# gmongaras/Stable-Diffusion-3-From-Scratch

Measured on AMD Instinct MI355X. Metric: train images/sec MMDiT-B 256^2 bf16, higher is better.
Workload: dtype bf16

## Files before the change

### stable-diffusion-3-from-scratch_amd/csrc/rowops.hip

```cpp
#include "common.h"
#include <float.h>

namespace {

constexpr float LN_EPS = 1e-5f;
constexpr float RMS_EPS = FLT_EPSILON;

__device__ __forceinline__ float bf16_round(float x) { return __builtin_bit_cast(float, pack_bf2(x, 0.f) << 16); }

template <int NITX, typename TO, typename TA, bool RES, bool MX = false>
__device__ __forceinline__ void ln_mod_fwd_body(int block, const float* __restrict__ x, const float* __restrict__ scale, const float* __restrict__ shift,
                                                int64_t ld_mod, int rows, int d, int rpb, TO* __restrict__ out,
                                                float* __restrict__ mean_o, float* __restrict__ rstd_o,
                                                const TA* __restrict__ acc, const float* __restrict__ gate, int64_t ld_gate, float* __restrict__ xo,
                                                unsigned char* __restrict__ mx_scales) {
  constexpr int NIT = NITX < 0 ? -NITX : NITX;
  constexpr bool EXACT = NITX < 0;
  const int lane = threadIdx.x & 63, row = block * 4 + (threadIdx.x >> 6);
  if (row >= rows) return;
  const int nch = d >> 2;
  const int b = row / rpb;
  const float* xr = x + (int64_t)row * d;
  float v[NIT][4];
  float s = 0.f;
// ... 194 lines not shown
    flush(dh, dshift + (int64_t)b * ld_dmod);
    if constexpr (GATED) {
      flush(sg, dgate + (int64_t)b * ld_dgate);
      if (dbias) flush(sb, dbias + (int64_t)b * ld_dbias);
    }
  }
}

struct LnBwdProb {
  const void* dout; const float* x; const float* mean; const float* rstd; const float* scale; int64_t ld_mod; const float* dres; int rpb, nchunk;
  float* dx; float* dscale; float* dshift; int64_t ld_dmod;
  const void* acc; const float* gate; int64_t ld_gate; void* dacc; float* dgate; int64_t ld_dgate; float* dbias; int64_t ld_dbias;
};
template <int NIT, typename TG, typename TA, bool GATED>
__global__ __launch_bounds__(256) void ln_mod_bwd_kernel(LnBwdProb p0, LnBwdProb p1, int nblk0, int d, int rch) {
  const bool first = (int)blockIdx.x < nblk0;
  const LnBwdProb& p = first ? p0 : p1;
  ln_mod_bwd_body<NIT, TG, TA, GATED>(first ? (int)blockIdx.x : (int)blockIdx.x - nblk0, (const TG*)p.dout, p.x, p.mean, p.rstd, p.scale, p.ld_mod, p.dres, d, p.rpb, p.nchunk,
                                      p.dx, p.dscale, p.dshift, p.ld_dmod, (const TA*)p.acc, p.gate, p.ld_gate, (TA*)p.dacc, p.dgate, p.ld_dgate, p.dbias, p.ld_dbias, rch);
}

template <int NITX, typename TI, typename TO>
__global__ __launch_bounds__(256) void text_rms_fwd_kernel(const TI* __restrict__ x, const float* __restrict__ w, const float* __restrict__ sp,
                                                           int rows, int cnt, int tokens, int off, int d, TO* __restrict__ out) {
  constexpr int NIT = NITX < 0 ? -NITX : NITX;
  constexpr bool EXACT = NITX < 0;
  const int lane = threadIdx.x & 63, m = blockIdx.x * 4 + (threadIdx.x >> 6);
  if (m >= rows) return;
  const int nch = d >> 2;
  const TI* xr = x + ((int64_t)(m / cnt) * tokens + off + m % cnt) * d;
  float v[NIT][4];
  float q = 0.f;
#pragma unroll
  for (int it = 0; it < NIT; it++) {
    int ch = lane + 64 * it;
    if (EXACT || ch < nch) { ld4(xr + ch * 4, v[it]); q += v[it][0] * v[it][0] + v[it][1] * v[it][1] + v[it][2] * v[it][2] + v[it][3] * v[it][3]; }
  }
  const float rinv = rsqrtf(wave_sum(q) / d + RMS_EPS);
  const float s = sp[0];
  TO* orow = out + (int64_t)m * d;
#pragma unroll
  for (int it = 0; it < NIT; it++) {
    int ch = lane + 64 * it;
    if (EXACT || ch < nch) {
      float wv[4], o[4];
      ld4(w + ch * 4, wv);
#pragma unroll
      for (int e = 0; e < 4; e++) o[e] = s * (v[it][e] * rinv * wv[e]);
      st4(orow + ch * 4, o);
    }
  }
}

#ifndef TRB_ROWS
#define TRB_ROWS 64
#endif
struct TextRmsBwdHalf { const void* dout; const float* w; const float* sp; int rows, cnt, off; float* dw; float* dsp; };
template <int NITX, typename TI, typename TG>
__global__ __launch_bounds__(512) void text_rms_bwd_kernel(TextRmsBwdHalf h0, TextRmsBwdHalf h1, const TI* __restrict__ x, int tokens, int d) {
  constexpr int NIT = NITX < 0 ? -NITX : NITX;
  constexpr bool EXACT = NITX < 0;
  const TextRmsBwdHalf& hp = blockIdx.y == 0 ? h0 : h1;
  const TG* __restrict__ dout = (const TG*)hp.dout;
  const float* __restrict__ w = hp.w;
  const float* __restrict__ sp = hp.sp;
  const int rows = hp.rows, cnt = hp.cnt, off = hp.off;
  float* __restrict__ dw = hp.dw;
  float* __restrict__ dsp = hp.dsp;
  __shared__ float red[NIT * 256];
  for (int c = threadIdx.x; c < NIT * 256; c += 512) red[c] = 0.f;
  __syncthreads();
  const int lane = threadIdx.x & 63, wave = threadIdx.x >> 6;
  const int nch = d >> 2;
  const float s = sp[0];
  float accw[NIT][4], wv[NIT][4];
  float accs = 0.f;
#pragma unroll
  for (int it = 0; it < NIT; it++) {
    int ch = lane + 64 * it;
    if (EXACT || ch < nch) ld4(w + ch * 4, wv[it]); else { wv[it][0] = wv[it][1] = wv[it][2] = wv[it][3] = 0.f; }
#pragma unroll
    for (int e = 0; e < 4; e++) accw[it][e] = 0.f;
  }
  for (int m = blockIdx.x * TRB_ROWS + wave; m < min(rows, (int)(blockIdx.x + 1) * TRB_ROWS); m += 8) {
    const TI* xr = x + ((int64_t)(m / cnt) * tokens + off + m % cnt) * d;
    float v[NIT][4];
    float q = 0.f;
#pragma unroll
    for (int it = 0; it < NIT; it++) {
      int ch = lane + 64 * it;
      if (EXACT || ch < nch) { ld4(xr + ch * 4, v[it]); q += v[it][0] * v[it][0] + v[it][1] * v[it][1] + v[it][2] * v[it][2] + v[it][3] * v[it][3]; }
    }
    const float rinv = rsqrtf(wave_sum(q) / d + RMS_EPS);
#pragma unroll
    for (int it = 0; it < NIT; it++) {
      int ch = lane + 64 * it;
      if (EXACT || ch < nch) {
        float dy[4];
        ld4(dout + (int64_t)m * d + ch * 4, dy);
#pragma unroll
        for (int e = 0; e < 4; e++) { float xn = v[it][e] * rinv; accw[it][e] += dy[e] * s * xn; accs += dy[e] * xn * wv[it][e]; }
      }
    }
  }
#pragma unroll
  for (int it = 0; it < NIT; it++) {
    const int ch = lane + 64 * it;
    if (EXACT || ch < nch) {
#pragma unroll
      for (int e = 0; e < 4; e++) atomicAdd(&red[ch * 4 + e], accw[it][e]);
    }
  }
  __syncthreads();
#ifndef TRB_NO_GLOBAL
  for (int c = threadIdx.x; c < d; c += 512) atomicAdd(dw + c, red[c]);
#else
  if (red[threadIdx.x] == 123.456f) dw[0] = 1.f;
#endif
  accs = wave_sum(accs);
#ifndef TRB_NO_DSP
  if (lane == 0) atomicAdd(dsp, accs);
#else
  if (accs == 123.456f) dsp[0] = 1.f;
#endif
}

__device__ __forceinline__ float group8_sum(float v) {
  v += __shfl_xor(v, 1, 64); v += __shfl_xor(v, 2, 64); v += __shfl_xor(v, 4, 64);
  return v;
}

template <typename TI>
__device__ __forceinline__ void qk_norm_rope_fwd_body(int bid, int rstride, const TI* __restrict__ qkv, const float* __restrict__ wq, const float* __restrict__ wk,
                                                      const float* __restrict__ rcos, const float* __restrict__ rsin,
                                                      int rows, int tokens, int heads, int s_total, int tok0,
                                                      bf16_t* __restrict__ Q, bf16_t* __restrict__ K, bf16_t* __restrict__ V) {
  const int hc = threadIdx.x % (8 * heads), part = threadIdx.x / (8 * heads), head = hc >> 3, chunk = hc & 7;
  bf16_t* obase = part == 0 ? Q : part == 1 ? K : V;
  float w[8];
#pragma unroll
  for (int e = 0; e < 8; e++) w[e] = 0.f;
  if (part < 2) ld8((part == 0 ? wq : wk) + chunk * 8, w);
  const bool same_token = rcos && rstride % tokens == 0;
  float cs[2][8], sn[2][8];
  if (same_token && part < 2) {
    const int n = bid % tokens;
    ld8(rcos + (int64_t)n * 64 + chunk * 8, cs[0]);
    ld8(rsin + (int64_t)n * 64 + chunk * 8, sn[0]);
#pragma unroll
    for (int e = 0; e < 8; e++) { cs[1][e] = cs[0][e]; sn[1][e] = sn[0][e]; }
  }
  for (int row0 = bid; row0 < rows; row0 += 2 * rstride) {
    float x[2][8];
#pragma unroll
    for (int k = 0; k < 2; k++) {
      const int row = min(row0 + k * rstride, rows - 1);
      ld8(qkv + (((int64_t)row * 3 + part) * heads + head) * 64 + chunk * 8, x[k]);
    }
    if (part < 2 && rcos && !same_token) {
#pragma unroll
      for (int k = 0; k < 2; k++) {
        const int n = min(row0 + k * rstride, rows - 1) % tokens;
        ld8(rcos + (int64_t)n * 64 + chunk * 8, cs[k]);
        ld8(rsin + (int64_t)n * 64 + chunk * 8, sn[k]);
      }
    }
#pragma unroll
    for (int k = 0; k < 2; k++) {
      const int row = row0 + k * rstride;
      if (row >= rows) break;
      const int n = row % tokens, b = row / tokens;
      if (part < 2) {
        float ss = 0.f;
#pragma unroll
        for (int e = 0; e < 8; e++) ss += x[k][e] * x[k][e];
        const float rinv = rsqrtf(group8_sum(ss) * (1.f / 64.f) + RMS_EPS);
#pragma unroll
// ... 216 lines not shown
        ld8_nt(qkv + ((((int64_t)pr * 2 + k) * 3 + part) * heads + head) * 64 + chunk * 8, x[k]);
        if (rcos) {
          ld8(rcos + (int64_t)(2 * j + k) * 64 + chunk * 8, cs[k]);
          ld8(rsin + (int64_t)(2 * j + k) * 64 + chunk * 8, sn[k]);
        }
      }
#pragma unroll
      for (int k = 0; k < 2; k++) {
        float ss = 0.f;
#pragma unroll
        for (int e = 0; e < 8; e++) ss += x[k][e] * x[k][e];
        const float rinv = rsqrtf(group8_sum(ss) * (1.f / 64.f) + RMS_EPS);
        if (rcos) {
#pragma unroll
          for (int p = 0; p < 4; p++) {
            float da = dz[k][2 * p], db = dz[k][2 * p + 1];
            dz[k][2 * p] = da * cs[k][2 * p] + db * sn[k][2 * p + 1];
            dz[k][2 * p + 1] = db * cs[k][2 * p + 1] - da * sn[k][2 * p];
          }
        }
        float dot = 0.f;
#pragma unroll
        for (int e = 0; e < 8; e++) {
          float xh = x[k][e] * rinv;
          aw[e] += dz[k][e] * xh;
          dz[k][e] *= w[e];
          dot += dz[k][e] * xh;
          x[k][e] = xh;
        }
        dot = group8_sum(dot) * (1.f / 64.f);
#pragma unroll
        for (int e = 0; e < 8; e++) dz[k][e] = rinv * (dz[k][e] - x[k][e] * dot);
      }
    }
#pragma unroll
    for (int k = 0; k < 2; k++) st8(dqkv + ((((int64_t)pr * 2 + k) * 3 + part) * heads + head) * 64 + chunk * 8, dz[k]);
  }
  if (part < 2) {
#pragma unroll
    for (int e = 0; e < 8; e++) atomicAdd(&sdw[part][chunk * 8 + e], aw[e]);
  }
  __syncthreads();
  for (int i = threadIdx.x; i < 128; i += blockDim.x) atomicAdd((i < 64 ? dwq : dwk) + (i & 63), sdw[i >> 6][i & 63]);
}
template <typename TG, typename TI, typename TO>
__global__ __launch_bounds__(512) void qk_merge_bwd_kernel(QkProb p0, QkProb p1, int g0, int heads, int s_total) {
  const bool first = (int)blockIdx.x < g0;
  const QkProb& p = first ? p0 : p1;
  qk_merge_bwd_body<TG, TI, TO>(first ? (int)blockIdx.x : (int)blockIdx.x - g0, first ? g0 : (int)gridDim.x - g0, (const TG*)p.dQ, (const TG*)p.dK, (const TG*)p.dV,
                                (const TI*)p.qkv, p.wq, p.wk, p.rcos, p.rsin, p.rows >> 1, p.tokens, heads, s_total, p.tok0, (TO*)p.dqkv, p.dwq, p.dwk);
}

constexpr int CO_RCH = 64;

__device__ __forceinline__ float gelu_f(float x) { return 0.5f * x * (1.f + erff(x * 0.70710678118654752440f)); }
__device__ __forceinline__ float gelu_grad_f(float x) {
  return 0.5f * (1.f + erff(x * 0.70710678118654752440f)) + x * 0.39894228040143267794f * __expf(-0.5f * x * x);
}

template <typename T, bool GELU, bool MX = false>
__global__ __launch_bounds__(256) void mlp_act_fwd_kernel(const T* __restrict__ gu, T* __restrict__ h, int rows, int hidden, unsigned char* __restrict__ mx_scales = nullptr) {
  const int tx = threadIdx.x & 31, ty = threadIdx.x >> 5;
  const int c = blockIdx.x * 256 + tx * 8;
  if (c >= hidden) return;
  const int64_t ldi = GELU ? hidden : 2 * (int64_t)hidden;
  const int rend = min(rows, (int)(blockIdx.y + 1) * CO_RCH);
  for (int r0 = blockIdx.y * CO_RCH + ty; r0 < rend; r0 += 16) {
    float g[2][8], u[2][8];
#pragma unroll
    for (int k = 0; k < 2; k++) {
      const int r = r0 + 8 * k;
      if (r < rend) {
        ld8(gu + r * ldi + c, g[k]);
        if constexpr (!GELU) ld8(gu + r * ldi + hidden + c, u[k]);
      }
    }
#pragma unroll
    for (int k = 0; k < 2; k++) {
      const int r = r0 + 8 * k;
      if (r >= rend) break;
      float o[8];
#pragma unroll
      for (int e = 0; e < 8; e++) o[e] = GELU ? gelu_f(g[k][e]) : silu_f(g[k][e]) * u[k][e];
      if constexpr (MX) {
        float amax = 0.f;
#pragma unroll
        for (int e = 0; e < 8; e++) { o[e] = bf16_round(o[e]); amax = fmaxf(amax, fabsf(o[e])); }
        amax = fmaxf(amax, __shfl_xor(amax, 1, 64));
        amax = fmaxf(amax, __shfl_xor(amax, 2, 64));
        float inv;
        const int ex = mx_exponent(amax, inv);
        *(uint2*)((unsigned char*)h + (int64_t)r * hidden + c) = make_uint2(mx_pack4(o, inv), mx_pack4(o + 4, inv));
        if ((tx & 3) == 0) mx_scales[mx_scale_index(r, c >> 5, rows)] = (unsigned char)(ex + 127);
      } else {
        st8(h + (int64_t)r * hidden + c, o);
      }
    }
  }
}

__device__ __forceinline__ void colsum_flush(float (&acc)[8], float* sbuf , float* dst, int c, int ncols) {
  const int tx = threadIdx.x & 127, ty = threadIdx.x >> 7;
  if (ty == 1) {
#pragma unroll
    for (int e = 0; e < 8; e++) sbuf[tx * 8 + e] = acc[e];
  }
  __syncthreads();
  if (ty == 0 && c < ncols) {
#pragma unroll
    for (int e = 0; e < 8; e++) atomicAdd(dst + c + e, acc[e] + sbuf[tx * 8 + e]);
  }
  __syncthreads();
}

constexpr int MB_RCH = 128;
template <typename T, bool GELU>
__device__ __forceinline__ void mlp_act_bwd_body(int by, const T* __restrict__ dh, const T* __restrict__ gu, T* __restrict__ dgu,
                                                 int rows, int hidden, float* __restrict__ dbias) {
  __shared__ float sbuf[8 * 256];
  const int tx = threadIdx.x & 31, ty = threadIdx.x >> 5;
  const int c = blockIdx.x * 256 + tx * 8;
  const bool act = c < hidden;
  const int64_t ldi = GELU ? hidden : 2 * (int64_t)hidden;
  float sg[8], su[8];
#pragma unroll
  for (int e = 0; e < 8; e++) { sg[e] = 0.f; su[e] = 0.f; }
  const int rend = min(rows, (by + 1) * MB_RCH);
  if (act) {
    for (int r0 = by * MB_RCH + ty; r0 < rend; r0 += 16) {
      float d[2][8], g[2][8], u[2][8];
#pragma unroll
      for (int k = 0; k < 2; k++) {
        const int r = r0 + 8 * k;
        if (r < rend) {
          ld8_nt(dh + (int64_t)r * hidden + c, d[k]);
          ld8_nt(gu + r * ldi + c, g[k]);
          if constexpr (!GELU) ld8_nt(gu + r * ldi + hidden + c, u[k]);
        }
      }
#pragma unroll
      for (int k = 0; k < 2; k++) {
        const int r = r0 + 8 * k;
        if (r >= rend) break;
        float og[8], ou[8];
        if constexpr (GELU) {
#pragma unroll
          for (int e = 0; e < 8; e++) { og[e] = d[k][e] * gelu_grad_f(g[k][e]); sg[e] += og[e]; }
          st8(dgu + r * ldi + c, og);
        } else {
#pragma unroll
          for (int e = 0; e < 8; e++) {
            swiglu_bwd_f(d[k][e], g[k][e], u[k][e], og[e], ou[e]);
            sg[e] += og[e]; su[e] += ou[e];
          }
          st8(dgu + r * ldi + c, og);
          st8(dgu + r * ldi + hidden + c, ou);
        }
      }
    }
  }
  if (dbias) {
    const int col = blockIdx.x * 256 + threadIdx.x;
#pragma unroll
    for (int which = 0; which < (GELU ? 1 : 2); which++) {
#pragma unroll
// ... 22 lines not shown
__global__ __launch_bounds__(256) void gate_res_bwd_kernel(const float* __restrict__ dy, const TA* __restrict__ acc, const float* __restrict__ gate, int64_t ld_gate,
                                                           int d, int rpb, int nchunk, TO* __restrict__ dacc,
                                                           float* __restrict__ dgate, int64_t ld_dgate, float* __restrict__ dbias, int64_t ld_dbias) {
  __shared__ float sbuf[8 * 256];
  const int tx = threadIdx.x & 31, ty = threadIdx.x >> 5;
  const int c = blockIdx.x * 256 + tx * 8;
  const bool act = c < d;
  const int b = blockIdx.y / nchunk, chunk = blockIdx.y % nchunk;
  float g[8], sgate[8], sb[8];
#pragma unroll
  for (int e = 0; e < 8; e++) { g[e] = 0.f; sgate[e] = 0.f; sb[e] = 0.f; }
  if (act) {
    ld8(gate + (int64_t)b * ld_gate + c, g);
    const int rend = min(rpb, (chunk + 1) * GR_RCH);
    for (int rl = chunk * GR_RCH + ty; rl < rend; rl += 16) {
      const int64_t row0 = (int64_t)b * rpb + rl, row1 = row0 + 8;
      const bool two = rl + 8 < rend;
      float dv0[8], av0[8], dv1[8], av1[8], o[8];
      ld8(dy + row0 * d + c, dv0);
      ld8(acc + row0 * d + c, av0);
      if (two) {
        ld8(dy + row1 * d + c, dv1);
        ld8(acc + row1 * d + c, av1);
      }
#pragma unroll
      for (int e = 0; e < 8; e++) { o[e] = dv0[e] * g[e]; sgate[e] += dv0[e] * av0[e]; sb[e] += o[e]; }
      st8(dacc + row0 * d + c, o);
      if (two) {
#pragma unroll
        for (int e = 0; e < 8; e++) { o[e] = dv1[e] * g[e]; sgate[e] += dv1[e] * av1[e]; sb[e] += o[e]; }
        st8(dacc + row1 * d + c, o);
      }
    }
  }
  const int col = blockIdx.x * 256 + threadIdx.x;
#pragma unroll
  for (int which = 0; which < 2; which++) {
    float* dst = which == 0 ? dgate + (int64_t)b * ld_dgate : (dbias ? dbias + (int64_t)b * ld_dbias : nullptr);
    if (!dst) break;
#pragma unroll
    for (int e = 0; e < 8; e++) sbuf[ty * 256 + tx * 8 + e] = which == 0 ? sgate[e] : sb[e];
    __syncthreads();
    if (col < d) {
      float s = 0.f;
#pragma unroll
      for (int r = 0; r < 8; r++) s += sbuf[r * 256 + threadIdx.x];
      atomicAdd(dst + col, s);
    }
    __syncthreads();
  }
}

template <typename T>
__global__ __launch_bounds__(256) void colsum_kernel(const T* __restrict__ x, int rows, int cols, int64_t ld, float* __restrict__ out, int rch) {
  __shared__ float sbuf[1024];
  const int tx = threadIdx.x & 127, ty = threadIdx.x >> 7;
  const int c = blockIdx.x * 1024 + tx * 8;
  float s[8];
#pragma unroll
  for (int e = 0; e < 8; e++) s[e] = 0.f;
  if (c < cols) {
    const int rend = min(rows, (int)(blockIdx.y + 1) * rch);
#pragma unroll 4
    for (int r = blockIdx.y * rch + ty; r < rend; r += 2) {
      float v[8];
      ld8(x + r * ld + c, v);
#pragma unroll
      for (int e = 0; e < 8; e++) s[e] += v[e];
    }
  }
  colsum_flush(s, sbuf, out, c, cols);
}

template <typename TG, typename TO>
__global__ __launch_bounds__(256) void silu_bwd_kernel(const TG* __restrict__ dy, const float* __restrict__ pre, TO* __restrict__ dpre, int rpg, int cols, float* __restrict__ dbias) {
  __shared__ float sb[4][64];
  const int cl = threadIdx.x & 63, rl = threadIdx.x >> 6;
  const int c = blockIdx.x * 64 + cl;
  const int r0 = blockIdx.y * rpg;
  float s = 0.f;
  if (c < cols) {
#pragma unroll 4
    for (int r = r0 + rl; r < r0 + rpg; r += 4) {
      const int64_t i = (int64_t)r * cols + c;
      const float p = pre[i], sig = sigmoid_f(p);
      const float g = io<TG>::ld(dy + i) * sig * (1.f + p * (1.f - sig));
      io<TO>::st(dpre + i, g);
      s += g;
    }
  }
  sb[rl][cl] = s;
  __syncthreads();
  if (rl == 0 && c < cols && dbias) dbias[(int64_t)blockIdx.y * cols + c] += sb[0][cl] + sb[1][cl] + sb[2][cl] + sb[3][cl];
}

template <typename TI, typename TO>
__global__ void cast_kernel(const TI* __restrict__ src, TO* __restrict__ dst, int64_t n) {
  const int64_t n8 = n >> 3;
  for (int64_t i = (int64_t)blockIdx.x * blockDim.x + threadIdx.x; i < n8; i += (int64_t)gridDim.x * blockDim.x) {
    float v[8];
    ld8(src + i * 8, v);
    st8(dst + i * 8, v);
  }
  if (blockIdx.x == 0 && threadIdx.x < (n & 7)) io<TO>::st(dst + n8 * 8 + threadIdx.x, io<TI>::ld(src + n8 * 8 + threadIdx.x));
}

template <typename TI, typename TO, bool TO_TOKENS>
__global__ void patch_kernel(const TI* __restrict__ src, TO* __restrict__ dst, int batch, int ch, int H, int W) {
  const int W2 = W >> 1, H2 = H >> 1;
  const int64_t total = (int64_t)batch * ch * H * W2;
  for (int64_t g = (int64_t)blockIdx.x * blockDim.x + threadIdx.x; g < total; g += (int64_t)gridDim.x * blockDim.x) {
    const int j = (int)(g % W2); int64_t r = g / W2;
    const int y = (int)(r % H); r /= H;
    const int c = (int)(r % ch); const int64_t b = r / ch;
    const int64_t img_off = ((b * ch + c) * H + y) * W + 2 * j;
    const int64_t tok_off = ((b * H2 + (y >> 1)) * W2 + j) * (int64_t)(ch * 4) + c * 4 + (y & 1) * 2;
    if (TO_TOKENS) { io<TO>::st(dst + tok_off, io<TI>::ld(src + img_off)); io<TO>::st(dst + tok_off + 1, io<TI>::ld(src + img_off + 1)); }
    else { io<TO>::st(dst + img_off, io<TI>::ld(src + tok_off)); io<TO>::st(dst + img_off + 1, io<TI>::ld(src + tok_off + 1)); }
  }
}

template <typename TO>
__global__ void time_embed_fwd_kernel(const float* __restrict__ t, const float* __restrict__ ts, const float* __restrict__ denom, int batch, int dim, TO* __restrict__ out) {
  const int i = blockIdx.x * blockDim.x + threadIdx.x, b = blockIdx.y;
  if (i >= dim) return;
  const float tau = t[b] * ts[0];
  const int half = dim >> 1;
  const float v = i < half ? sinf(tau / denom[2 * i]) : cosf(tau / denom[2 * (i - half) + 1]);
  io<TO>::st(out + (int64_t)b * dim + i, v);
}

template <typename TG>
__global__ __launch_bounds__(256) void time_embed_bwd_kernel(const TG* __restrict__ dout, const float* __restrict__ t, const float* __restrict__ ts,
                                                             const float* __restrict__ denom, int batch, int dim, float* __restrict__ dts) {
  __shared__ float red[4];
  const int b = blockIdx.x;
  const float tau = t[b] * ts[0];
  const int half = dim >> 1;
  float s = 0.f;
  for (int i = threadIdx.x; i < dim; i += 256) {
    const float g = io<TG>::ld(dout + (int64_t)b * dim + i);
    if (i < half) { const float dn = denom[2 * i]; s += g * cosf(tau / dn) / dn; }
    else { const float dn = denom[2 * (i - half) + 1]; s -= g * sinf(tau / dn) / dn; }
  }
  s = wave_sum(s);
  if ((threadIdx.x & 63) == 0) red[threadIdx.x >> 6] = s;
  __syncthreads();
  if (threadIdx.x == 0) atomicAdd(dts, (red[0] + red[1] + red[2] + red[3]) * t[b]);
}

inline int nit_for(int d) { return (d / 4 + 63) / 64; }
inline int grid_cap(int64_t n, int bs) { int64_t g = (n + bs - 1) / bs; return (int)(g < 1 ? 1 : g > 4096 ? 4096 : g); }

}

#define NIT_CASE(n, ...)                                                        \
  { if (d == (n) * 256) { constexpr int NIT = -(n); __VA_ARGS__; } else { constexpr int NIT = (n); __VA_ARGS__; } }
#define NIT_SWITCH(nit, ...)                                    \
  do {                                                          \
    if (nit <= 1) NIT_CASE(1, __VA_ARGS__)                      \
    else if (nit <= 2) NIT_CASE(2, __VA_ARGS__)                 \
    else if (nit <= 3) NIT_CASE(3, __VA_ARGS__)                 \
    else if (nit <= 4) NIT_CASE(4, __VA_ARGS__)                 \
    else if (nit <= 6) NIT_CASE(6, __VA_ARGS__)                 \
    else if (nit <= 9) NIT_CASE(9, __VA_ARGS__)                 \
    else if (nit <= 12) NIT_CASE(12, __VA_ARGS__)               \
    else NIT_CASE(16, __VA_ARGS__)                              \
  } while (0)

#define LN_FWD_NIT (NIT < 0 ? -NIT : NIT)

extern "C" int mmdit_abi_version(void) { return MMDIT_ABI_VERSION; }
extern "C" int mmdit_struct_size(int which) {
  switch (which) {
    case 0: return (int)sizeof(mmdit_gemm_args);
    case 1: return (int)sizeof(mmdit_ln_fwd_problem);
    case 2: return (int)sizeof(mmdit_ln_bwd_problem);
    case 3: return (int)sizeof(mmdit_qk_problem);
    case 4: return (int)sizeof(mmdit_mlp_bwd_problem);
    case 5: return (int)sizeof(mmdit_adamw_tensor);
    case 6: return (int)sizeof(mmdit_cast_tensor);
    case 7: return (int)sizeof(mmdit_qk_epilogue);
    default: return -1;
  }
}
extern "C" const char* mmdit_build_arch(void) { return "gfx950"; }

static int ln_mod_fwd_launch(const mmdit_ln_fwd_problem* probs, int count, int d, int out_dtype, unsigned char* mx_scales, hipStream_t s) {
  MMDIT_CHECK_ARG(probs && count >= 1 && count <= 2 && d > 0 && d % 4 == 0 && d <= 4096);
  const bool res = probs[0].acc != nullptr;
  LnFwdProb q[2] = {};
  int nb[2] = {0, 0};
  for (int i = 0; i < count; i++) {
    const mmdit_ln_fwd_problem* p = probs + i;
    MMDIT_CHECK_ARG((p->acc != nullptr) == res);
    MMDIT_CHECK_ARG(p->x && p->scale && p->shift && p->out && p->mean && p->rstd && p->rows > 0 && p->rows_per_batch > 0 && p->ld_mod % 4 == 0);
    if (res) MMDIT_CHECK_ARG(p->gate && p->x_out && p->ld_gate % 4 == 0);
    q[i] = LnFwdProb{p->x, p->scale, p->shift, p->ld_mod, p->rows, p->rows_per_batch, p->out, p->mean, p->rstd, p->acc, p->gate, p->ld_gate, p->x_out, mx_scales};
    nb[i] = (p->rows + 3) / 4;
  }
  const int nit = nit_for(d);
  dim3 grid(nb[0] + nb[1]);
#define LNL(TO, TA, RES, MX) NIT_SWITCH(nit, hipLaunchKernelGGL((ln_mod_fwd_kernel<LN_FWD_NIT, TO, TA, RES, MX>), grid, dim3(256), 0, s, q[0], q[1], nb[0], d))
  if (mx_scales) { if (res) { LNL(unsigned char, bf16_t, true, true); } else { LNL(unsigned char, bf16_t, false, true); } }
  else if (out_dtype == MMDIT_BF16) { if (res) { LNL(bf16_t, bf16_t, true, false); } else { LNL(bf16_t, bf16_t, false, false); } }
  else if (out_dtype == MMDIT_F32) { if (res) { LNL(float, float, true, false); } else { LNL(float, float, false, false); } }
  else return MMDIT_ERR_DTYPE;
#undef LNL
  return mmdit_launch_status();
}

extern "C" int mmdit_ln_modulate_fwd(const mmdit_ln_fwd_problem* probs, int count, int d, int acc_dtype, int out_dtype, mmdit_stream_t stream) {
  MMDIT_CHECK_ARG(probs && count >= 1 && (!probs[0].acc || acc_dtype == out_dtype));
  return ln_mod_fwd_launch(probs, count, d, out_dtype, nullptr, (hipStream_t)stream);
}

extern "C" int mmdit_ln_modulate_fwd_mx(const float* x, const void* acc, int acc_dtype, const float* gate, int64_t ld_gate, float* x_out,
                                        const float* scale, const float* shift, int64_t ld_mod, int rows, int d, int rpb,
                                        void* q_fp8, void* scales_e8m0, float* mean, float* rstd, mmdit_stream_t stream) {
  MMDIT_CHECK_ARG(scales_e8m0 && d % 64 == 0 && (!acc || acc_dtype == MMDIT_BF16));
  const mmdit_ln_fwd_problem p = {x, acc, gate, ld_gate, x_out, scale, shift, ld_mod, rows, rpb, q_fp8, mean, rstd};
  return ln_mod_fwd_launch(&p, 1, d, MMDIT_FP8, (unsigned char*)scales_e8m0, (hipStream_t)stream);
}

extern "C" int mmdit_gate_residual_fwd(const float* x, const void* acc, int acc_dtype, const float* gate, int64_t ld_gate, int rows, int d, int rpb,
                                       float* out, mmdit_stream_t stream) {
  MMDIT_CHECK_ARG(x && acc && gate && out && rows > 0 && d > 0 && d % 4 == 0 && rpb > 0 && ld_gate % 4 == 0);
  hipStream_t s = (hipStream_t)stream;
  dim3 grid(grid_cap((int64_t)rows * (d / 4), 256));
  if (acc_dtype == MMDIT_BF16) hipLaunchKernelGGL((gate_residual_fwd_kernel<bf16_t>), grid, dim3(256), 0, s, x, (const bf16_t*)acc, gate, ld_gate, rows, d, rpb, out);
  else if (acc_dtype == MMDIT_F32) hipLaunchKernelGGL((gate_residual_fwd_kernel<float>), grid, dim3(256), 0, s, x, (const float*)acc, gate, ld_gate, rows, d, rpb, out);
  else return MMDIT_ERR_DTYPE;
  return mmdit_launch_status();
}

static int ln_bwd_one_round_rch(const mmdit_ln_bwd_problem* a, const mmdit_ln_bwd_problem* b, int d, int dout_dtype, bool gated) {
  auto wgs = [&](int r) { return (long)(a->rows / a->rows_per_batch) * ((a->rows_per_batch + r - 1) / r) + (long)(b->rows / b->rows_per_batch) * ((b->rows_per_batch + r - 1) / r); };
  const int nit_ = nit_for(d), nit_abs = nit_ < 0 ? -nit_ : nit_;
  int per_cu = nit_abs <= 3 ? 4 : nit_abs == 4 ? 3 : 2, cus = 256;
  {
    static int occ[64][17][2][2], cu_count[64];
    const int dev = mmdit_current_device(), ti = dout_dtype == MMDIT_BF16 ? 0 : 1, gi = gated ? 1 : 0, ni = nit_abs > 16 ? 16 : nit_abs;
    if (!cu_count[dev]) {
      int n = 0;
      cu_count[dev] = (hipDeviceGetAttribute(&n, hipDeviceAttributeMultiprocessorCount, dev) == hipSuccess && n > 0) ? n : 256;
    }
    cus = cu_count[dev];
    if (!occ[dev][ni][ti][gi]) {
      int nbq = 0;
      hipError_t e = hipErrorUnknown;
#define LNQ(T, G) NIT_SWITCH(nit_, e = hipOccupancyMaxActiveBlocksPerMultiprocessor(&nbq, (const void*)ln_mod_bwd_kernel<(NIT < 0 ? -NIT : NIT), T, T, G>, 256, 0))
      if (dout_dtype == MMDIT_BF16) { if (gated) { LNQ(bf16_t, true); } else { LNQ(bf16_t, false); } }
      else if (dout_dtype == MMDIT_F32) { if (gated) { LNQ(float, true); } else { LNQ(float, false); } }
#undef LNQ
      occ[dev][ni][ti][gi] = (e == hipSuccess && nbq > 0) ? nbq : 8;
    }
    per_cu = per_cu < occ[dev][ni][ti][gi] ? per_cu : occ[dev][ni][ti][gi];
  }
  const long slots = (long)cus * per_cu;
  if (wgs(LN_BWD_RCH) > slots && wgs(LN_BWD_RCH) <= 2 * slots)
    for (int r = LN_BWD_RCH + 4; r <= 64; r += 4)
      if (wgs(r) <= slots) return r;
  return LN_BWD_RCH;
}

extern "C" int mmdit_ln_modulate_bwd(const mmdit_ln_bwd_problem* probs, int count, int d, int dout_dtype, mmdit_stream_t stream) {
  MMDIT_CHECK_ARG(probs && count >= 1 && count <= 2 && d > 0 && d % 4 == 0 && d <= 4096);
  const bool gated = probs[0].acc != nullptr;
  for (int i = 0; i < count; i++) {
    const mmdit_ln_bwd_problem* p = probs + i;
    MMDIT_CHECK_ARG((p->acc != nullptr) == gated);
    MMDIT_CHECK_ARG(p->dout && p->x && p->mean && p->rstd && p->scale && p->dx && p->dscale && p->dshift && p->rows > 0 && p->rows_per_batch > 0 &&
                    p->rows % p->rows_per_batch == 0 && p->ld_mod % 4 == 0);
    if (gated) MMDIT_CHECK_ARG(p->gate && p->dacc && p->dgate && p->ld_gate % 4 == 0);
  }
  if (dout_dtype != MMDIT_BF16 && dout_dtype != MMDIT_F32) return MMDIT_ERR_DTYPE;
  const int rch = count == 2 ? ln_bwd_one_round_rch(probs, probs + 1, d, dout_dtype, gated) : LN_BWD_RCH;
  LnBwdProb q[2] = {};
  int nb[2] = {0, 0};
  for (int i = 0; i < count; i++) {
    const mmdit_ln_bwd_problem* p = probs + i;
    const int nchunk = (p->rows_per_batch + rch - 1) / rch;
    nb[i] = (p->rows / p->rows_per_batch) * nchunk;
    q[i] = LnBwdProb{p->dout, p->x, p->mean, p->rstd, p->scale, p->ld_mod, p->dres, p->rows_per_batch, nchunk, p->dx, p->dscale, p->dshift, p->ld_dmod,
                     p->acc, p->gate, p->ld_gate, p->dacc, p->dgate, p->ld_dgate, p->dbias, p->ld_dbias};
  }
  hipStream_t s = (hipStream_t)stream;
  const int nit = nit_for(d);
  dim3 grid(nb[0] + nb[1]);
#define LNL(T, G) NIT_SWITCH(nit, hipLaunchKernelGGL((ln_mod_bwd_kernel<(NIT < 0 ? -NIT : NIT), T, T, G>), grid, dim3(256), 0, s, q[0], q[1], nb[0], d, rch))
  if (dout_dtype == MMDIT_BF16) { if (gated) { LNL(bf16_t, true); } else { LNL(bf16_t, false); } }
  else { if (gated) { LNL(float, true); } else { LNL(float, false); } }
#undef LNL
  return mmdit_launch_status();
}

extern "C" int mmdit_text_rmsnorm_fwd(const void* x, int x_dtype, const float* w1, const float* w2, const float* s1, const float* s2,
                                      int batch, int tokens, int split, int d, void* out1, void* out2, int out_dtype, mmdit_stream_t stream) {
  MMDIT_CHECK_ARG(x && w1 && w2 && s1 && s2 && out1 && out2 && batch > 0 && split > 0 && split < tokens && d % 4 == 0 && d <= 4096);
  hipStream_t s = (hipStream_t)stream;
  const int nit = nit_for(d);
  for (int half = 0; half < 2; half++) {
    const int cnt = half ? tokens - split : split, off = half ? split : 0, rows = batch * cnt;
    const float* w = half ? w2 : w1; const float* sp = half ? s2 : s1; void* out = half ? out2 : out1;
    dim3 grid((rows + 3) / 4);
#define TRF(TI, TO) NIT_SWITCH(nit, hipLaunchKernelGGL((text_rms_fwd_kernel<LN_FWD_NIT, TI, TO>), grid, dim3(256), 0, s, (const TI*)x, w, sp, rows, cnt, tokens, off, d, (TO*)out))
    if (x_dtype == MMDIT_F32 && out_dtype == MMDIT_F32) { TRF(float, float); }
    else if (x_dtype == MMDIT_F32 && out_dtype == MMDIT_BF16) { TRF(float, bf16_t); }
    else if (x_dtype == MMDIT_BF16 && out_dtype == MMDIT_BF16) { TRF(bf16_t, bf16_t); }
    else if (x_dtype == MMDIT_BF16 && out_dtype == MMDIT_F32) { TRF(bf16_t, float); }
    else return MMDIT_ERR_DTYPE;
#undef TRF
  }
  return mmdit_launch_status();
}

extern "C" int mmdit_text_rmsnorm_bwd(const void* dout1, const void* dout2, int dout_dtype, const void* x, int x_dtype,
                                      const float* w1, const float* w2, const float* s1, const float* s2, int batch, int tokens, int split, int d,
                                      float* dw1, float* dw2, float* ds1, float* ds2, mmdit_stream_t stream) {
  MMDIT_CHECK_ARG(dout1 && dout2 && x && w1 && w2 && s1 && s2 && dw1 && dw2 && ds1 && ds2 && batch > 0 && split > 0 && split < tokens && d % 4 == 0 && d <= 4096);
  hipStream_t s = (hipStream_t)stream;
  const int nit = nit_for(d);
  TextRmsBwdHalf h[2];
  int maxrows = 0;
  for (int half = 0; half < 2; half++) {
    const int cnt = half ? tokens - split : split, rows = batch * cnt;
    h[half] = TextRmsBwdHalf{half ? dout2 : dout1, half ? w2 : w1, half ? s2 : s1, rows, cnt, half ? split : 0, half ? dw2 : dw1, half ? ds2 : ds1};
    maxrows = rows > maxrows ? rows : maxrows;
  }
  dim3 grid((maxrows + TRB_ROWS - 1) / TRB_ROWS, 2);
#define TRB(TI, TG) NIT_SWITCH(nit, hipLaunchKernelGGL((text_rms_bwd_kernel<NIT, TI, TG>), grid, dim3(512), 0, s, h[0], h[1], (const TI*)x, tokens, d))
  if (x_dtype == MMDIT_F32 && dout_dtype == MMDIT_F32) { TRB(float, float); }
  else if (x_dtype == MMDIT_F32 && dout_dtype == MMDIT_BF16) { TRB(float, bf16_t); }
  else if (x_dtype == MMDIT_BF16 && dout_dtype == MMDIT_BF16) { TRB(bf16_t, bf16_t); }
  else if (x_dtype == MMDIT_BF16 && dout_dtype == MMDIT_F32) { TRB(bf16_t, float); }
  else return MMDIT_ERR_DTYPE;
#undef TRB
  return mmdit_launch_status();
}

static int qk_bwd_rl(int heads, int min_rows) {
  static const int env = [] { const char* e = mmdit_exp_env("MMDIT_QK_RL"); return e ? atoi(e) : 0; }();
  int rl = 1024 / (24 * heads);
  if (env > 0 && env < rl) rl = env;
  if (rl < 1 || min_rows < 2048) rl = 1;
  return rl;
}
static int qk_bwd_grid(int rows, int tokens, bool rope, int& rl) {
  static const int lanes_max = [] { const char* e = mmdit_exp_env("MMDIT_QK_LANES"); return e ? atoi(e) : 768; }();
  if (rl == 1) {
    int g = rows < 512 ? rows : 512;
    if (rope && tokens <= 1024 && rows >= tokens) g = (g / tokens > 0 ? g / tokens : 1) * tokens;
    return g;
  }
  if (!rope) return lanes_max / rl;
  if (tokens > lanes_max) return tokens <= 2048 && tokens % rl == 0 ? tokens / rl : lanes_max / rl;
  int k = lanes_max / tokens;
  while (k > 1 && (k * tokens) % rl) k--;
  if ((k * tokens) % rl) return lanes_max / rl;
  return k * tokens / rl;
}

static int qk_check(const mmdit_qk_problem* p, int s_total, bool bwd) {
  if (!(p->qkv && p->wq && p->wk && p->tokens > 0 && p->tok0 >= 0 && p->tok0 + p->tokens <= s_total && (p->rope_cos == nullptr) == (p->rope_sin == nullptr))) return MMDIT_ERR_ARG;
  if (bwd && !(p->dqkv && p->dwq && p->dwk)) return MMDIT_ERR_ARG;
  return 0;
}
static int qk_merge_check(const mmdit_qk_problem* p, int s_total, bool bwd) {
  if (int e = qk_check(p, s_total, bwd)) return e;
  if ((p->tokens | p->tok0 | s_total) & 1) return MMDIT_ERR_SHAPE;
  return 0;
}
static int qk_list(const mmdit_qk_problem* probs, int count, int batch, int heads, int s_total, int max_threads, bool merge,
                   bool bwd, const void* dQ, const void* dK, const void* dV, QkProb (&q)[2]) {
  MMDIT_CHECK_ARG(probs && count >= 1 && count <= 2 && batch > 0 && heads > 0 && 24 * heads <= max_threads && (!bwd || (dQ && dK && dV)));
  for (int i = 0; i < count; i++) {
    const mmdit_qk_problem* p = probs + i;
    if (int e = merge ? qk_merge_check(p, s_total, bwd) : qk_check(p, s_total, bwd)) return e;
    q[i] = QkProb{p->qkv, p->wq, p->wk, p->rope_cos, p->rope_sin, batch * p->tokens, p->tokens, p->tok0, dQ, dK, dV,
                  bwd ? p->dqkv : nullptr, bwd ? p->dwq : nullptr, bwd ? p->dwk : nullptr};
  }
  return 0;
}
static int qk_bwd_combo(int dq_dtype, int qkv_dtype, int dqkv_dtype) {
// ... 146 lines not shown
namespace {
template <typename T>
__global__ __launch_bounds__(256) void flow_loss_partial_kernel(const float* __restrict__ v, const T* __restrict__ x0, const T* __restrict__ eps, int64_t n8, float coef2,
                                                                float* __restrict__ dv, float* __restrict__ partials) {
  float s = 0.f;
  for (int64_t i = (int64_t)blockIdx.x * 256 + threadIdx.x; i < n8; i += (int64_t)gridDim.x * 256) {
    float a[8], b[8], c[8], g[8];
    ld8(v + i * 8, a);
    ld8(x0 + i * 8, b);
    ld8(eps + i * 8, c);
#pragma unroll
    for (int e = 0; e < 8; e++) {
      float lab = c[e] - b[e];
      if (sizeof(T) == 2) lab = bf2f(f2bf(lab));
      const float d = a[e] - lab;
      s += d * d;
      g[e] = coef2 * d;
    }
    if (dv) st8(dv + i * 8, g);
  }
  __shared__ float sm[4];
  s = wave_sum(s);
  if ((threadIdx.x & 63) == 0) sm[threadIdx.x >> 6] = s;
  __syncthreads();
  if (threadIdx.x == 0) partials[blockIdx.x] = ((sm[0] + sm[1]) + sm[2]) + sm[3];
}
__global__ __launch_bounds__(64) void flow_loss_final_kernel(const float* __restrict__ partials, int count, float coef, float* __restrict__ loss) {
  float s = 0.f;
  for (int i = threadIdx.x; i < count; i += 64) s += partials[i];
  s = wave_sum(s);
  if (threadIdx.x == 0) loss[0] = s * coef;
}
}

extern "C" int mmdit_flow_loss(const float* v, const void* x0, const void* eps, int in_dtype, int64_t n, float coef, float* dv, float* partials,
                               float* loss, mmdit_stream_t stream) {
  MMDIT_CHECK_ARG(v && x0 && eps && partials && loss && n > 0 && n % 8 == 0);
  const int64_t n8 = n / 8;
  const int grid = (int)((n8 + 255) / 256 < 256 ? (n8 + 255) / 256 : 256);
  hipStream_t s = (hipStream_t)stream;
  if (in_dtype == MMDIT_BF16)
    hipLaunchKernelGGL((flow_loss_partial_kernel<bf16_t>), dim3(grid), dim3(256), 0, s, v, (const bf16_t*)x0, (const bf16_t*)eps, n8, 2.f * coef, dv, partials);
  else if (in_dtype == MMDIT_F32)
    hipLaunchKernelGGL((flow_loss_partial_kernel<float>), dim3(grid), dim3(256), 0, s, v, (const float*)x0, (const float*)eps, n8, 2.f * coef, dv, partials);
  else
    return MMDIT_ERR_DTYPE;
  hipLaunchKernelGGL(flow_loss_final_kernel, dim3(1), dim3(64), 0, s, (const float*)partials, grid, coef, loss);
  return mmdit_launch_status();
}

extern "C" int mmdit_colsum(const void* x, int dtype, int rows, int cols, int64_t ld, float* out, mmdit_stream_t stream) {
  MMDIT_CHECK_ARG(x && out && rows > 0 && cols > 0 && cols % 8 == 0 && ld % 8 == 0);
  hipStream_t s = (hipStream_t)stream;
  const int rch = rows <= 256 ? 8 : CO_RCH;
  dim3 grid((cols + 1023) / 1024, (rows + rch - 1) / rch);
  if (dtype == MMDIT_BF16) hipLaunchKernelGGL((colsum_kernel<bf16_t>), grid, dim3(256), 0, s, (const bf16_t*)x, rows, cols, ld, out, rch);
  else if (dtype == MMDIT_F32) hipLaunchKernelGGL((colsum_kernel<float>), grid, dim3(256), 0, s, (const float*)x, rows, cols, ld, out, rch);
  else return MMDIT_ERR_DTYPE;
  return mmdit_launch_status();
}

namespace {
template <typename TI>
__global__ __launch_bounds__(256) void fp8_amax_kernel(const TI* __restrict__ x, int64_t n8, float* __restrict__ amax) {
  float m = 0.f;
  for (int64_t i = (int64_t)blockIdx.x * 256 + threadIdx.x; i < n8; i += (int64_t)gridDim.x * 256) {
    float v[8];
    ld8(x + i * 8, v);
#pragma unroll
    for (int e = 0; e < 8; e++) m = fmaxf(m, fabsf(v[e]));
  }
  __shared__ float sm[4];
  m = wave_max(m);
  if ((threadIdx.x & 63) == 0) sm[threadIdx.x >> 6] = m;
  __syncthreads();
  if (threadIdx.x == 0) atomicMax((unsigned int*)amax, __float_as_uint(fmaxf(fmaxf(sm[0], sm[1]), fmaxf(sm[2], sm[3]))));
}
template <typename TI>
__global__ __launch_bounds__(256) void fp8_quant_kernel(const TI* __restrict__ x, int64_t n8, const float* __restrict__ amax, uint2* __restrict__ q, float* __restrict__ scale) {
  const float a = fmaxf(amax[0], 1e-12f), s = 448.f / a;
  if (blockIdx.x == 0 && threadIdx.x == 0) scale[0] = a / 448.f;
  for (int64_t i = (int64_t)blockIdx.x * 256 + threadIdx.x; i < n8; i += (int64_t)gridDim.x * 256) {
    float v[8];
    ld8(x + i * 8, v);
#pragma unroll
    for (int e = 0; e < 8; e++) v[e] = fminf(fmaxf(v[e] * s, -448.f), 448.f);
    int lo = 0, hi = 0;
    lo = __builtin_amdgcn_cvt_pk_fp8_f32(v[0], v[1], lo, false);
    lo = __builtin_amdgcn_cvt_pk_fp8_f32(v[2], v[3], lo, true);
    hi = __builtin_amdgcn_cvt_pk_fp8_f32(v[4], v[5], hi, false);
    hi = __builtin_amdgcn_cvt_pk_fp8_f32(v[6], v[7], hi, true);
    q[i] = make_uint2((unsigned)lo, (unsigned)hi);
  }
}
template <typename TI>
__global__ __launch_bounds__(256) void fp8_quant_delayed_kernel(const TI* __restrict__ x, int64_t n8, float* __restrict__ state, int phase, float margin,
                                                                uint2* __restrict__ q) {
  __shared__ float sm[4];
  const float a = fmaxf(state[phase % 3] * margin, 1e-12f), s = 448.f / a;
  if (blockIdx.x == 0 && threadIdx.x == 0) { state[3] = a / 448.f; state[(phase + 2) % 3] = 0.f; }
  float m = 0.f;
  for (int64_t i = (int64_t)blockIdx.x * 256 + threadIdx.x; i < n8; i += (int64_t)gridDim.x * 256) {
    float v[8];
    ld8(x + i * 8, v);
#pragma unroll
    for (int e = 0; e < 8; e++) { m = fmaxf(m, fabsf(v[e])); v[e] = fminf(fmaxf(v[e] * s, -448.f), 448.f); }
    int lo = 0, hi = 0;
    lo = __builtin_amdgcn_cvt_pk_fp8_f32(v[0], v[1], lo, false);
    lo = __builtin_amdgcn_cvt_pk_fp8_f32(v[2], v[3], lo, true);
    hi = __builtin_amdgcn_cvt_pk_fp8_f32(v[4], v[5], hi, false);
// ... 127 lines not shown
```

Before: 2407.

## Size text RMS backward and colsum grids from CU count, restructure reductions

The text RMSNorm backward kernel now takes its rows-per-block from the device CU count instead of a fixed 64. It issues all x and dout loads before reducing, using nontemporal loads for dout, and sums the per-wave scale gradient in shared memory so each block does one global atomic instead of one per wave. The colsum kernel is rewritten to split columns into narrow slabs with many row lanes per block, unroll its loads four deep, and cap the number of row chunks, which limits global atomics. The aim is better memory-level parallelism and fewer atomics in small reduction kernels, at the cost of heuristic grid sizing that may not suit every shape.

```diff
diff --git a/stable-diffusion-3-from-scratch_amd/csrc/rowops.hip b/stable-diffusion-3-from-scratch_amd/csrc/rowops.hip
--- a/stable-diffusion-3-from-scratch_amd/csrc/rowops.hip
+++ b/stable-diffusion-3-from-scratch_amd/csrc/rowops.hip
@@ -270,12 +270,19 @@
   }
 }
 
-#ifndef TRB_ROWS
-#define TRB_ROWS 64
-#endif
+constexpr int TRB_WAVES = 8, TRB_MIN_ROWS = 40;
+__device__ __forceinline__ void ld4_raw_nt(const float* p, f32x4& r) { r = __builtin_nontemporal_load((const f32x4*)p); }
+__device__ __forceinline__ void ld4_raw_nt(const bf16_t* p, u32x2& r) { r = __builtin_nontemporal_load((const u32x2*)p); }
+__device__ __forceinline__ void widen4(const f32x4& r, float (&v)[4]) { v[0] = r[0]; v[1] = r[1]; v[2] = r[2]; v[3] = r[3]; }
+__device__ __forceinline__ void widen4(const u32x2& r, float (&v)[4]) {
+  v[0] = __builtin_bit_cast(float, r[0] << 16); v[1] = __builtin_bit_cast(float, r[0] & 0xffff0000u);
+  v[2] = __builtin_bit_cast(float, r[1] << 16); v[3] = __builtin_bit_cast(float, r[1] & 0xffff0000u);
+}
+template <typename T> struct Raw4 { using type = f32x4; };
+template <> struct Raw4<bf16_t> { using type = u32x2; };
 struct TextRmsBwdHalf { const void* dout; const float* w; const float* sp; int rows, cnt, off; float* dw; float* dsp; };
 template <int NITX, typename TI, typename TG>
-__global__ __launch_bounds__(512) void text_rms_bwd_kernel(TextRmsBwdHalf h0, TextRmsBwdHalf h1, const TI* __restrict__ x, int tokens, int d) {
+__global__ __launch_bounds__(TRB_WAVES * 64) void text_rms_bwd_kernel(TextRmsBwdHalf h0, TextRmsBwdHalf h1, const TI* __restrict__ x, int tokens, int d, int rpw) {
   constexpr int NIT = NITX < 0 ? -NITX : NITX;
   constexpr bool EXACT = NITX < 0;
   const TextRmsBwdHalf& hp = blockIdx.y == 0 ? h0 : h1;
@@ -285,8 +292,11 @@
   const int rows = hp.rows, cnt = hp.cnt, off = hp.off;
   float* __restrict__ dw = hp.dw;
   float* __restrict__ dsp = hp.dsp;
+  const int mend = min(rows, (int)(blockIdx.x + 1) * rpw);
+  if ((int)blockIdx.x * rpw >= mend) return;
   __shared__ float red[NIT * 256];
-  for (int c = threadIdx.x; c < NIT * 256; c += 512) red[c] = 0.f;
+  __shared__ float sred[TRB_WAVES];
+  for (int c = threadIdx.x; c < NIT * 256; c += TRB_WAVES * 64) red[c] = 0.f;
   __syncthreads();
   const int lane = threadIdx.x & 63, wave = threadIdx.x >> 6;
   const int nch = d >> 2;
@@ -300,14 +310,26 @@
 #pragma unroll
     for (int e = 0; e < 4; e++) accw[it][e] = 0.f;
   }
-  for (int m = blockIdx.x * TRB_ROWS + wave; m < min(rows, (int)(blockIdx.x + 1) * TRB_ROWS); m += 8) {
+  for (int m = blockIdx.x * rpw + wave; m < mend; m += TRB_WAVES) {
     const TI* xr = x + ((int64_t)(m / cnt) * tokens + off + m % cnt) * d;
+    const TG* dr = dout + (int64_t)m * d;
     float v[NIT][4];
-    float q = 0.f;
+    typename Raw4<TG>::type dyr[NIT];
 #pragma unroll
     for (int it = 0; it < NIT; it++) {
       int ch = lane + 64 * it;
-      if (EXACT || ch < nch) { ld4(xr + ch * 4, v[it]); q += v[it][0] * v[it][0] + v[it][1] * v[it][1] + v[it][2] * v[it][2] + v[it][3] * v[it][3]; }
+      if (EXACT || ch < nch) ld4(xr + ch * 4, v[it]);
+    }
+#pragma unroll
+    for (int it = 0; it < NIT; it++) {
+      int ch = lane + 64 * it;
+      if (EXACT || ch < nch) ld4_raw_nt(dr + ch * 4, dyr[it]);
+    }
+    float q = 0.f;
+#pragma unroll
+    for (int it = 0; it < NIT; it++) {
+      int ch = lane + 64 * it;
+      if (EXACT || ch < nch) q += v[it][0] * v[it][0] + v[it][1] * v[it][1] + v[it][2] * v[it][2] + v[it][3] * v[it][3];
     }
     const float rinv = rsqrtf(wave_sum(q) / d + RMS_EPS);
 #pragma unroll
@@ -315,7 +337,7 @@
       int ch = lane + 64 * it;
       if (EXACT || ch < nch) {
         float dy[4];
-        ld4(dout + (int64_t)m * d + ch * 4, dy);
+        widen4(dyr[it], dy);
 #pragma unroll
         for (int e = 0; e < 4; e++) { float xn = v[it][e] * rinv; accw[it][e] += dy[e] * s * xn; accs += dy[e] * xn * wv[it][e]; }
       }
@@ -329,18 +351,16 @@
       for (int e = 0; e < 4; e++) atomicAdd(&red[ch * 4 + e], accw[it][e]);
     }
   }
+  accs = wave_sum(accs);
+  if (lane == 0) sred[wave] = accs;
   __syncthreads();
-#ifndef TRB_NO_GLOBAL
-  for (int c = threadIdx.x; c < d; c += 512) atomicAdd(dw + c, red[c]);
-#else
-  if (red[threadIdx.x] == 123.456f) dw[0] = 1.f;
-#endif
-  accs = wave_sum(accs);
-#ifndef TRB_NO_DSP
-  if (lane == 0) atomicAdd(dsp, accs);
-#else
-  if (accs == 123.456f) dsp[0] = 1.f;
-#endif
+  for (int c = threadIdx.x; c < d; c += TRB_WAVES * 64) atomicAdd(dw + c, red[c]);
+  if (threadIdx.x == 0) {
+    float a = sred[0];
+#pragma unroll
+    for (int k = 1; k < TRB_WAVES; k++) a += sred[k];
+    atomicAdd(dsp, a);
+  }
 }
 
 __device__ __forceinline__ float group8_sum(float v) {
@@ -663,6 +683,7 @@
 }
 
 constexpr int CO_RCH = 64;
+constexpr int CO_SLAB_GROUPS = 8, CO_UNROLL = 4, CO_WG_PER_CU = 4, CO_MAX_ADDERS = 128;
 
 __device__ __forceinline__ float gelu_f(float x) { return 0.5f * x * (1.f + erff(x * 0.70710678118654752440f)); }
 __device__ __forceinline__ float gelu_grad_f(float x) {
@@ -708,20 +729,6 @@
       }
     }
   }
-}
-
-__device__ __forceinline__ void colsum_flush(float (&acc)[8], float* sbuf , float* dst, int c, int ncols) {
-  const int tx = threadIdx.x & 127, ty = threadIdx.x >> 7;
-  if (ty == 1) {
-#pragma unroll
-    for (int e = 0; e < 8; e++) sbuf[tx * 8 + e] = acc[e];
-  }
-  __syncthreads();
-  if (ty == 0 && c < ncols) {
-#pragma unroll
-    for (int e = 0; e < 8; e++) atomicAdd(dst + c + e, acc[e] + sbuf[tx * 8 + e]);
-  }
-  __syncthreads();
 }
 
 constexpr int MB_RCH = 128;
@@ -850,24 +857,39 @@
 }
 
 template <typename T>
-__global__ __launch_bounds__(256) void colsum_kernel(const T* __restrict__ x, int rows, int cols, int64_t ld, float* __restrict__ out, int rch) {
-  __shared__ float sbuf[1024];
-  const int tx = threadIdx.x & 127, ty = threadIdx.x >> 7;
-  const int c = blockIdx.x * 1024 + tx * 8;
+__global__ __launch_bounds__(256) void colsum_kernel(const T* __restrict__ x, int rows, int cols, int64_t ld, float* __restrict__ out, int rch, int ncg, int rl) {
+  __shared__ float sbuf[256 * 8];
+  const int ty = threadIdx.x / ncg, tx = threadIdx.x - ty * ncg;
+  const int c = (blockIdx.x * ncg + tx) * 8;
   float s[8];
 #pragma unroll
   for (int e = 0; e < 8; e++) s[e] = 0.f;
-  if (c < cols) {
+  if (ty < rl && c < cols) {
     const int rend = min(rows, (int)(blockIdx.y + 1) * rch);
-#pragma unroll 4
-    for (int r = blockIdx.y * rch + ty; r < rend; r += 2) {
-      float v[8];
-      ld8(x + r * ld + c, v);
-#pragma unroll
-      for (int e = 0; e < 8; e++) s[e] += v[e];
-    }
-  }
-  colsum_flush(s, sbuf, out, c, cols);
+    const int64_t step = rl * ld;
+    int r = blockIdx.y * rch + ty;
+    const T* p = x + r * ld + c;
+    for (; r < rend; r += CO_UNROLL * rl, p += CO_UNROLL * step) {
+      float v[CO_UNROLL][8];
+#pragma unroll
+      for (int k = 0; k < CO_UNROLL; k++) ld8(r + k * rl < rend ? p + k * step : p, v[k]);
+#pragma unroll
+      for (int k = 0; k < CO_UNROLL; k++) {
+        const bool in = r + k * rl < rend;
+#pragma unroll
+        for (int e = 0; e < 8; e++) s[e] += in ? v[k][e] : 0.f;
+      }
+    }
+  }
+#pragma unroll
+  for (int e = 0; e < 8; e++) sbuf[threadIdx.x * 8 + e] = s[e];
+  __syncthreads();
+  const int w = ncg * 8, col = blockIdx.x * w + threadIdx.x;
+  if ((int)threadIdx.x < w && col < cols) {
+    float a = 0.f;
+    for (int l = 0; l < rl; l++) a += sbuf[l * w + threadIdx.x];
+    atomicAdd(out + col, a);
+  }
 }
 
 template <typename TG, typename TO>
@@ -949,6 +971,15 @@
 
 inline int nit_for(int d) { return (d / 4 + 63) / 64; }
 inline int grid_cap(int64_t n, int bs) { int64_t g = (n + bs - 1) / bs; return (int)(g < 1 ? 1 : g > 4096 ? 4096 : g); }
+inline int device_cu_count() {
+  static int cu_count[64];
+  const int dev = mmdit_current_device();
+  if (!cu_count[dev]) {
+    int n = 0;
+    cu_count[dev] = (hipDeviceGetAttribute(&n, hipDeviceAttributeMultiprocessorCount, dev) == hipSuccess && n > 0) ? n : 256;
+  }
+  return cu_count[dev];
+}
 
 }
 
@@ -1037,13 +1068,9 @@
   const int nit_ = nit_for(d), nit_abs = nit_ < 0 ? -nit_ : nit_;
   int per_cu = nit_abs <= 3 ? 4 : nit_abs == 4 ? 3 : 2, cus = 256;
   {
-    static int occ[64][17][2][2], cu_count[64];
+    static int occ[64][17][2][2];
     const int dev = mmdit_current_device(), ti = dout_dtype == MMDIT_BF16 ? 0 : 1, gi = gated ? 1 : 0, ni = nit_abs > 16 ? 16 : nit_abs;
-    if (!cu_count[dev]) {
-      int n = 0;
-      cu_count[dev] = (hipDeviceGetAttribute(&n, hipDeviceAttributeMultiprocessorCount, dev) == hipSuccess && n > 0) ? n : 256;
-    }
-    cus = cu_count[dev];
+    cus = device_cu_count();
     if (!occ[dev][ni][ti][gi]) {
       int nbq = 0;
       hipError_t e = hipErrorUnknown;
@@ -1126,8 +1153,11 @@
     h[half] = TextRmsBwdHalf{half ? dout2 : dout1, half ? w2 : w1, half ? s2 : s1, rows, cnt, half ? split : 0, half ? dw2 : dw1, half ? ds2 : ds1};
     maxrows = rows > maxrows ? rows : maxrows;
   }
-  dim3 grid((maxrows + TRB_ROWS - 1) / TRB_ROWS, 2);
-#define TRB(TI, TG) NIT_SWITCH(nit, hipLaunchKernelGGL((text_rms_bwd_kernel<NIT, TI, TG>), grid, dim3(512), 0, s, h[0], h[1], (const TI*)x, tokens, d))
+  const int slots = device_cu_count();
+  int rpw = ((batch * tokens + slots - 1) / slots + TRB_WAVES - 1) / TRB_WAVES * TRB_WAVES;
+  rpw = rpw < TRB_MIN_ROWS ? TRB_MIN_ROWS : rpw;
+  dim3 grid((maxrows + rpw - 1) / rpw, 2);
+#define TRB(TI, TG) NIT_SWITCH(nit, hipLaunchKernelGGL((text_rms_bwd_kernel<NIT, TI, TG>), grid, dim3(TRB_WAVES * 64), 0, s, h[0], h[1], (const TI*)x, tokens, d, rpw))
   if (x_dtype == MMDIT_F32 && dout_dtype == MMDIT_F32) { TRB(float, float); }
   else if (x_dtype == MMDIT_F32 && dout_dtype == MMDIT_BF16) { TRB(float, bf16_t); }
   else if (x_dtype == MMDIT_BF16 && dout_dtype == MMDIT_BF16) { TRB(bf16_t, bf16_t); }
@@ -1380,10 +1410,13 @@
 extern "C" int mmdit_colsum(const void* x, int dtype, int rows, int cols, int64_t ld, float* out, mmdit_stream_t stream) {
   MMDIT_CHECK_ARG(x && out && rows > 0 && cols > 0 && cols % 8 == 0 && ld % 8 == 0);
   hipStream_t s = (hipStream_t)stream;
-  const int rch = rows <= 256 ? 8 : CO_RCH;
-  dim3 grid((cols + 1023) / 1024, (rows + rch - 1) / rch);
-  if (dtype == MMDIT_BF16) hipLaunchKernelGGL((colsum_kernel<bf16_t>), grid, dim3(256), 0, s, (const bf16_t*)x, rows, cols, ld, out, rch);
-  else if (dtype == MMDIT_F32) hipLaunchKernelGGL((colsum_kernel<float>), grid, dim3(256), 0, s, (const float*)x, rows, cols, ld, out, rch);
+  const int groups = cols / 8, nslab = (groups + CO_SLAB_GROUPS - 1) / CO_SLAB_GROUPS, ncg = (groups + nslab - 1) / nslab, rl = 256 / ncg;
+  int chunks = (CO_WG_PER_CU * device_cu_count() + nslab - 1) / nslab;
+  chunks = chunks > CO_MAX_ADDERS ? CO_MAX_ADDERS : chunks;
+  const int rch = ((rows + chunks - 1) / chunks + rl - 1) / rl * rl;
+  dim3 grid(nslab, (rows + rch - 1) / rch);
+  if (dtype == MMDIT_BF16) hipLaunchKernelGGL((colsum_kernel<bf16_t>), grid, dim3(256), 0, s, (const bf16_t*)x, rows, cols, ld, out, rch, ncg, rl);
+  else if (dtype == MMDIT_F32) hipLaunchKernelGGL((colsum_kernel<float>), grid, dim3(256), 0, s, (const float*)x, rows, cols, ld, out, rch, ncg, rl);
   else return MMDIT_ERR_DTYPE;
   return mmdit_launch_status();
 }
```

After: 2420, median of 6. About the same (+0.5%).
